# adthoms/dcora

Hardware: AMD Instinct MI355X
Metric: RBCD iterations/sec, sphere2500 5-agent split (higher is better)
Workload: dtype f64

## Files before the change

### dcora_amd/capi.py

```python
import ctypes as C
import os
import subprocess

import numpy as np

_HERE = os.path.dirname(os.path.abspath(__file__))
LIB_PATH = os.path.join(_HERE, "lib", "libdcora_hip.so")
HEADER_PATH = os.path.join(os.path.dirname(_HERE), "include", "dcora_hip.h")


class DcoraError(RuntimeError):
    def __init__(self, status, msg):
        super().__init__("dcora status %d: %s" % (status, msg))
        self.status = status


class Dims(C.Structure):
    _fields_ = [("r", C.c_int), ("d", C.c_int), ("n", C.c_int), ("l", C.c_int), ("b", C.c_int), ("layout", C.c_int)]


LAYOUT_AUTO, LAYOUT_SE, LAYOUT_RA = 0, 1, 2


class ROptParams(C.Structure):
# ... 167 lines not shown
    "dcora_exchange_info": (C.c_int, [_vp, _dp]),
    "dcora_exchange_link_report": (C.c_int, [_vp, _dp]),
    "dcora_exchange_post": (C.c_int, [_vp, _ip, C.c_int]),
    "dcora_exchange_wait": (C.c_int, [_vp, _ip, C.c_int]),
    "dcora_exchange_evaluate": (C.c_int, [_vp, _PD, _PD, _vp, _PI]),
    "dcora_exchange_rbcd_iterate": (C.c_int, [_vp, C.c_int, _PD, _PD, _vp, _PI]),
    "dcora_exchange_rbcd_tick": (C.c_int, [_vp, _ip, C.c_int, C.c_int]),
    "dcora_exchange_run_coloured": (C.c_int, [_vp, C.c_int, C.c_double, _PI, _vp, _vp]),
    "dcora_exchange_set_X": (C.c_int, [_vp, _dp]),
    "dcora_exchange_gather_X": (C.c_int, [_vp, _dp]),
    "dcora_exchange_barrier": (C.c_int, [_vp]),
    "dcora_exchange_all_ready": (C.c_int, [_vp, C.c_int, _PI]),
    "dcora_exchange_update_weights": (C.c_int, [_vp, C.c_int, _vp]),
    "dcora_exchange_set_weights": (C.c_int, [_vp, _dp]),
    "dcora_exchange_get_weights": (C.c_int, [_vp, _dp]),
    "dcora_exchange_certify": (C.c_int, [_vp, C.c_int, _vp, _vp, _vp, C.c_double, _PI, _PD, _PD, _dp,
                                         C.POINTER(C.c_longlong), _PI]),
    "dcora_exchange_host_selftest": (C.c_int, [C.c_char_p, C.c_int, C.c_int, C.c_int, C.c_int, _PD]),
    "dcora_debug_exchange_leave_stale": (C.c_int, [C.c_char_p, C.c_int, C.c_int]),
    "dcora_debug_exchange_probe_fault": (C.c_int, [C.c_int]),
    "dcora_cert_prepare": (C.c_int, [C.POINTER(Dims), _ip, _ip, C.c_int, C.c_int]),
    "dcora_debug_tcg_run_fault": (C.c_int, [C.c_int]),
    "dcora_debug_tcg_run_fault_at": (C.c_int, [C.c_int, C.c_int]),
    "dcora_problem_solver_info": (C.c_int, [_vp, _dp]),
    "dcora_ra_rbcd_create": (C.c_int, [_vp, C.POINTER(RbcdOptions), C.POINTER(_vp)]),
    "dcora_ra_rbcd_destroy": (C.c_int, [_vp]),
    "dcora_ra_rbcd_info": (C.c_int, [_vp, _PI, _vp]),
    "dcora_ra_rbcd_set_X": (C.c_int, [_vp, _dp]),
    "dcora_ra_rbcd_get_X": (C.c_int, [_vp, _dp]),
    "dcora_ra_rbcd_iterate": (C.c_int, [_vp, C.c_int, _PD, _PD, _vp, _PI]),
    "dcora_ra_rbcd_evaluate": (C.c_int, [_vp, _PD, _PD, _vp, _PI]),
    "dcora_ra_rbcd_run": (C.c_int, [_vp, C.c_int, C.c_double, _PI, _vp, _vp, _vp]),
    "dcora_ra_rbcd_iterate_set": (C.c_int, [_vp, _ip, C.c_int, C.c_int]),
    "dcora_ra_rbcd_set_acceleration": (C.c_int, [_vp, C.c_int]),
    "dcora_ra_rbcd_agent_colours": (C.c_int, [_vp, _ip, _PI]),
    "dcora_ra_rbcd_run_coloured": (C.c_int, [_vp, C.c_int, C.c_double, _PI, _vp, _vp]),
    "dcora_ra_rbcd_last_result": (C.c_int, [_vp, C.POINTER(ROptResult)]),
    "dcora_problem_time_qapply": (C.c_int, [_vp, C.c_int, _PD, _PD]),
    "dcora_problem_time_qapply_rotating": (C.c_int, [C.POINTER(_vp), C.c_int, C.c_int, _PD]),
    "dcora_problem_qapply_info": (C.c_int, [_vp, _dp]),
    "dcora_problem_time_precond": (C.c_int, [_vp, C.c_int, _PD, _PD]),
    "dcora_problem_precond_info": (C.c_int, [_vp, _dp]),
    "dcora_precond_cache_info": (C.c_int, [_dp]),
    "dcora_precond_cache_clear": (C.c_int, []),
    "dcora_robust_params_default": (None, [C.POINTER(RobustParams)]),
    "dcora_robust_weights": (C.c_int, [C.POINTER(RobustParams), C.c_int, C.c_int, _dp, _dp]),
# ... 58 lines not shown
```

### dcora_amd/csrc/capi.hip

```cpp
#include <cstdio>
#include <cstring>
#include <new>

#include "../../include/dcora_hip.h"
#include "cert.h"
#include "device_chol.h"
#include "device_problem.h"
#include "host_graph.h"
#include "host_threads.h"
#include "ra_rbcd.h"
#include "rbcd.h"
#include "precond_cache.h"
#include "exchange.h"
#include "host_robust.h"
#include "robust.h"
#include "round.h"

namespace dcora {
const std::string &get_last_error();
}
using namespace dcora;

struct dcora_problem_s {
  DeviceProblem p;
// ... 245 lines not shown
    info[2] = P.has_bsr ? (double)P.Qb.nblocks : 0.0;
    info[3] = P.has_bsr ? P.Qb.nblocks * (8.0 * (P.m.d + 1) * (P.m.d + 1) + 4.0) + 4.0 * (P.m.n + 1)
                        : 12.0 * P.Q.nnz + 4.0 * (P.m.k + 1);
    return DCORA_OK;
  });
}

int dcora_problem_solver_info(dcora_problem_t p, double *info) {
  return abi_call({p, info}, [&]() -> int {
    const DeviceProblem &P = p->p;
    info[0] = !P.use_pc() ? 0 : (P.tcg_run_ok ? 2 : 1);
    return DCORA_OK;
  });
}
int dcora_debug_tcg_run_fault(int runs) {
  g_tcg_run_fault_skip.store(0);
  g_tcg_run_fault.store(runs < 0 ? 0 : runs);
  return DCORA_OK;
}
int dcora_debug_tcg_run_fault_at(int skip, int runs) {
  g_tcg_run_fault_skip.store(skip < 0 ? 0 : skip);
  g_tcg_run_fault.store(runs < 0 ? 0 : runs);
  return DCORA_OK;
}
int dcora_problem_time_precond(dcora_problem_t p, int reps, double *avg_ms, double *bytes) {
  return abi_call({p, avg_ms, bytes}, [&] { return p->p.time_precond(reps, avg_ms, bytes); });
}
int dcora_problem_precond_info(dcora_problem_t p, double *info) {
  return abi_call({p, info}, [&]() -> int {
    const DeviceProblem &P = p->p;
    info[0] = !P.has_precond ? 0 : (P.sparse_precond ? 2 : 1);
    info[1] = !P.has_precond ? 0 : (P.sparse_precond ? P.sp.launches() : 1);
    info[2] = (double)P.precond_nnzL;
    info[3] = P.precond_setup_ms;
    info[4] = !P.has_precond ? 0 : (P.sparse_precond ? P.sp.weights_per_apply : (double)P.m.k * P.m.k);
    return DCORA_OK;
  });
}

int dcora_debug_sparse_weights_digest(dcora_problem_t p, double *out4) {
  return abi_call({p, out4}, [&]() -> int {
    const DeviceProblem &P = p->p;
    if (!P.sparse_precond || !P.sp.im) return bad("the problem has no sparse preconditioner");
    const DevBuf<double> &v = P.sp.im->vals;
    std::vector<double> h(v.n);
    DCORA_HIP(hipSetDevice(P.device));
// ... 1472 lines not shown
```

### dcora_amd/csrc/kernels.h

```cpp
#pragma once
#include <hip/hip_runtime.h>

#include <atomic>
#include <climits>
#include <vector>

namespace dcora {

constexpr int kMaxPartials = 1024;
constexpr int kBsrMaxGrid = 4096;
constexpr int kBlock = 256;
constexpr int kSpmmTile = 1536;

struct ManiDesc {
  int r, d, n, l, b, k, se;
  __host__ __device__ int rot_col(int i) const { return se ? i * (d + 1) : i * d; }
  __host__ __device__ int sphere_col(int i) const { return d * n + i; }
  __host__ __device__ int num_euc() const { return se ? n : n + b; }
  __host__ __device__ int euc_col(int e) const { return se ? e * (d + 1) + d : d * n + l + e; }
};
inline ManiDesc make_mani(int r, int d, int n, int l, int b, int layout = 0) {
  ManiDesc m;
  m.r = r; m.d = d; m.n = n; m.l = l; m.b = b;
  m.se = (layout == 2) ? 0 : ((l == 0 && b == 0) ? 1 : 0);
// ... 159 lines not shown
bool fused_supported(const ManiDesc &m);
bool group_supported(const ManiDesc &m);
int fused_pose_blocks(const ManiDesc &m);
int fused_nsplit(const ManiDesc &m);
int fused_precond_grid(const ManiDesc &m);
int fused_update_grid(const ManiDesc &m);
int launch_fused_hess(hipStream_t st, const ManiDesc &m, const CsrDev &Q, const double *z, const double *d_old,
                       double *d_new, Buf2 X, Buf2 S, double *Hd, const double *p3, int np3, double *p1,
                       SolverCtl *ctl, int seq, int iter,
                      const BsrDev *Ab = nullptr );
void launch_fused_precond(hipStream_t st, const ManiDesc &m, int ldm, const double *Minv, Buf2 grad,
                          const double *delta, const double *Hd, double *eta, double *Heta, const double *res_old,
                          double *res_new, double *Zpart, const double *p1, int np1, double *p2, SolverCtl *ctl,
                          HostFlags *hf, int seq, int iter, int first, SpFold sf = SpFold());
int fused_pc_blocks(const ManiDesc &m);
bool tcg_run_supported(const ManiDesc &m, int ldm, int cus, int max_rows_nnz);
int tcg_run_sync_words();
extern std::atomic<int> g_tcg_run_fault;
extern std::atomic<int> g_tcg_run_fault_skip;
int tcg_run_max_rows_nnz(const ManiDesc &m, const int *rowptr);
int launch_tcg_run(hipStream_t st, const ManiDesc &m, int ldm, const double *Minv, const CsrDev &Q, Buf2 grad, Buf2 X,
                   Buf2 S, double *d0, double *d1, double *Hd, double *eta, double *Heta, double *z, double *p1r,
                   double *p3, double *pC, unsigned *sync, SolverCtl *ctl, HostFlags *hf, int seq);
bool fused_pc_preferred(const ManiDesc &m, int ldm);
bool fused_pc_ready(const ManiDesc &m, int ldm);
int launch_fused_pc(hipStream_t st, const ManiDesc &m, int ldm, const double *Minv, Buf2 grad, Buf2 X,
                    const double *delta, const double *Hd, double *eta, double *Heta, const double *res_old,
                    double *res_new, double *z, const double *p1, int np1, double *p3, SolverCtl *ctl, HostFlags *hf,
                    int seq, int iter, int first, double *pC = nullptr );
void launch_fused_finish(hipStream_t st, const ManiDesc &m, Buf2 X, const double *Zpart, const double *res,
                         double *z, const double *p2, int np2, double *p3, SolverCtl *ctl, HostFlags *hf, int seq,
                         int iter, int first, int nsplit = -1 , SpFold sf = SpFold(),
                         double *zraw = nullptr );
int launch_fused_grad_bsr(hipStream_t st, int r, int d, const BsrDev &A, Buf2 X, const double *G, Buf2 EG, Buf2 RG, Buf2 S,
                          int sel, double *pA, double *pB, double *posenorm, Gate g,
                          const int *agent_start = nullptr, int agents = 0, int *wg_per_agent = nullptr);
int launch_fused_grad(hipStream_t st, const ManiDesc &m, const CsrDev &Q, Buf2 X, const double *G, Buf2 EG, Buf2 RG,
                      Buf2 Sblk, int sel, double *pA, double *pB, double *posenorm, Gate g,
                      const GradRide *ride = nullptr);
int launch_g_rgrad(hipStream_t st, const ManiDesc &m, Buf2 X, Buf2 EG, Buf2 RG, Buf2 Sblk, int sel, double *partials,
                   double *posenorm, Gate g);
void launch_ctl_init(hipStream_t st, SolverCtl *c, double tol, double Delta, double maxDelta, int max_outer,
                     int stop_on_accept, int max_inner);
void launch_eval_finish(hipStream_t st, int R, const int *pose_start, const double *posenorm, const double *pA,
                        int npA, EvalOut *out_dev, int seq, double *split_scratch = nullptr, int nposes = 0,
                        const double *agent_partials = nullptr, int wg_per_agent = 0);
// ... 84 lines not shown
```

### dcora_amd/csrc/solver_fused.hip

```cpp
#include <algorithm>
#include <stdexcept>
#include <atomic>
#include <type_traits>
#include <vector>
#include <cstdlib>
#include <cstring>

#include "kernels.h"
#include "tcg_rules.h"

namespace dcora {

namespace {

constexpr int GW = 8;

__device__ __forceinline__ double f_partial4_load(const double *__restrict__ p, int np) {
  const int l = (int)(threadIdx.x & 63u);
  const double a = (l < np) ? p[l] : 0.0, b = (l + 64 < np) ? p[l + 64] : 0.0;
  const double c = (l + 128 < np) ? p[l + 128] : 0.0, d = (l + 192 < np) ? p[l + 192] : 0.0;
  return (a + b) + (c + d);
}
__device__ __forceinline__ int f_partial_index(int np) { return np <= 64 ? (int)(threadIdx.x & 63u) : (int)threadIdx.x; }
__device__ __forceinline__ double f_partial_total(double v, int np, double *sm) {
// ... 904 lines not shown
  for (int a = 0; a < DH; ++a) acc += Zr.e[a] * Rr.e[a];
  const double tot = block_sum(acc, s_red);
  if (threadIdx.x == 0) p3[blockIdx.x] = tot;
  if (blockIdx.x == 0 && threadIdx.x == 0) {
    if (!first && iter + 1 >= c_max_inner) tcg_end_run_at_cap(ctl, hf, seq, iter + 1);
    host_store(&hf->last_seq_done, seq);
  }
}

typedef unsigned pc_v4u __attribute__((ext_vector_type(4)));
__device__ __forceinline__ double2 pc_ld16(__amdgpu_buffer_rsrc_t rs, unsigned voff, unsigned soff) {
  const pc_v4u v = __builtin_amdgcn_raw_buffer_load_b128(rs, voff, soff, 0);
  return __builtin_bit_cast(double2, v);
}
__device__ __forceinline__ double row16_sum_dpp(double v) {
  v += dpp_move<0xB1>(v);
  v += dpp_move<0x4E>(v);
  v += dpp_move<0x141>(v);
  v += dpp_move<0x140>(v);
  return v;
}
constexpr int kPcBlock = 256;
constexpr int kPcNW = kPcBlock / 64;
constexpr int kPcSB = 25;
constexpr int kPcLoads = 32;

template <int D, int PB, int R, bool MULTI>
__global__ __launch_bounds__(kPcBlock) void k_fused_pc(ManiDesc m, int ldm, int chk, const double *__restrict__ Minv,
                                                       Buf2 gradb, Buf2 Xb, const double *__restrict__ delta,
                                                       const double *__restrict__ Hd, double *__restrict__ eta,
                                                       double *__restrict__ Heta, const double *__restrict__ res_old,
                                                       double *__restrict__ res_new, double *__restrict__ z,
                                                       const double *__restrict__ p1, int np1,
                                                       double *__restrict__ p3, SolverCtl *ctl, HostFlags *hf, int seq,
                                                       int iter, int first, double *__restrict__ pC) {
  constexpr int DH = D + 1, NR = PB * DH, RM = R ? R : 8;
  constexpr int MB = kPcLoads / NR;
  extern __shared__ double s_res[];
  __shared__ double s_P[NR * RM + 1][4 * kPcNW];
  __shared__ double s_Z[NR * RM + 1], s_R[NR * RM];
  __shared__ double s_red[16];
  const int par = iter & 1;
  const int st_o = ctl->outer_done_stamp, st_t = ctl->tcg_done_stamp, cur = ctl->cur & 1;
  const double c_zr = ctl->z_r[par], c_dPd = ctl->d_Pd[par], c_ePe = ctl->e_Pe[par], c_ePd = ctl->e_Pd[par],
               c_Delta = ctl->Delta, c_ngf = ctl->ngf, c_n0 = ctl->norm_r0;
  const int c_max_inner = ctl->max_inner;
// ... 257 lines not shown

constexpr int kRunShards = 32, kRunCopies = 64, kRunStride = 32;
constexpr int kRunSyncWords = (kRunShards + 1 + kRunCopies + 1) * kRunStride;
constexpr int kRunQCap = 1024;
struct TcgRunArgs {
  ManiDesc m;
  int ldm;
  const double *Minv;
  CsrDev Q;
  Buf2 grad, X, S;
  double *d0, *d1, *Hd, *eta, *Heta, *z, *p1r, *p3, *pC;
  unsigned *sync;
  SolverCtl *ctl;
  HostFlags *hf;
  int seq, pbA;
  int fault;
#ifdef DCORA_RUN_STAMPS
  long long *stamps;
#endif
};
#ifdef DCORA_RUN_STAMPS
#define RUN_STAMP(i)                                                            \
  do {                                                                          \
    if (a.stamps && blockIdx.x == 0 && threadIdx.x == 0 && (i) < 64) a.stamps[(i)] = wall_clock64(); \
  } while (0)
#else
#define RUN_STAMP(i) \
  do {                \
  } while (0)
#endif
__device__ __forceinline__ double ld_coh(const double *p) {
  return __hip_atomic_load(p, __ATOMIC_RELAXED, __HIP_MEMORY_SCOPE_AGENT);
}
__device__ __forceinline__ void st_coh(double *p, double v) {
  __hip_atomic_store(p, v, __ATOMIC_RELAXED, __HIP_MEMORY_SCOPE_AGENT);
}
__device__ __forceinline__ double2 pc_ld16_coh(__amdgpu_buffer_rsrc_t rs, unsigned voff, unsigned soff) {
  const pc_v4u v = __builtin_amdgcn_raw_buffer_load_b128(rs, voff, soff, 16);
  return __builtin_bit_cast(double2, v);
}
constexpr unsigned kRunAbortBit = 0x80000000u;
__device__ __forceinline__ bool run_grid_step(unsigned *sync, unsigned step, int *s_ok) {
  __builtin_amdgcn_s_waitcnt(0);
  __syncthreads();
  if (threadIdx.x == 0) {
    unsigned *shard = sync, *top = sync + kRunShards * kRunStride, *done = top + kRunStride,
             *abort_w = done + kRunCopies * kRunStride;
    const int i = blockIdx.x, G = gridDim.x, sh = i % kRunShards;
    const unsigned in_shard = (unsigned)((G - sh + kRunShards - 1) / kRunShards), want = step + 1;
    const unsigned shards_used = (unsigned)(G < kRunShards ? G : kRunShards);
    const unsigned a = __hip_atomic_fetch_add(shard + sh * kRunStride, 1u, __ATOMIC_RELAXED, __HIP_MEMORY_SCOPE_AGENT);
    if (a + 1 == want * in_shard) {
      const unsigned b = __hip_atomic_fetch_add(top, 1u, __ATOMIC_RELAXED, __HIP_MEMORY_SCOPE_AGENT);
// ... 25 lines not shown
                                                     __HIP_MEMORY_SCOPE_AGENT)) {
              gave_up = true;
              break;
            }
          }
          if (gave_up) {
            __hip_atomic_store(abort_w, 1u, __ATOMIC_RELAXED, __HIP_MEMORY_SCOPE_AGENT);
            ok = 0;
            break;
          }
          t0 = wall_clock64();
        }
      }
    }
    *s_ok = ok;
  }
  __syncthreads();
  return *s_ok != 0;
}

template <int D, int R, int NS>
__global__ __launch_bounds__(kPcBlock) void k_tcg_run(TcgRunArgs a) {
  constexpr int DH = D + 1, PB = 2, NR = PB * DH, RM = R;
  extern __shared__ double s_res[];
  __shared__ double s_P[NR * RM + 1][4 * kPcNW];
  __shared__ double s_Z[NR * RM + 1], s_R[NR * RM], s_W[NR * RM], s_D[NR * RM], s_H[NR * RM];
  __shared__ double s_red[16];
  __shared__ int s_ci[kRunQCap];
  __shared__ double s_v[kRunQCap];
  __shared__ int s_ok;
  SolverCtl *ctl = a.ctl;
  const int seq = a.seq;
  RUN_STAMP(0);
  const int st_o = ctl->outer_done_stamp, cur = ctl->cur & 1;
  if (seq > st_o) return;
  const double c_Delta = ctl->Delta, c_ngf = ctl->ngf;
  const int c_max_inner = ctl->max_inner;
  const ManiDesc m = a.m;
  constexpr int r = R;
  const int k = m.k, ldm = a.ldm;
  const int pose0 = blockIdx.x * PB;
  const int npose = min(PB, m.n - pose0);
  const int j0 = pose0 * DH, nrow = npose * DH;
  const int wave = threadIdx.x >> 6, lane = threadIdx.x & 63;
  const int wave_u = __builtin_amdgcn_readfirstlane(wave);
  const int e = threadIdx.x;
  const bool own = e < nrow * r;
  const size_t oown = (size_t)j0 * r + e;
  const int lc = e / r, t = e - lc * r;
  const int g = threadIdx.x >> 3, tt = threadIdx.x & (GW - 1);
  const bool pact = (g < npose) && (tt < r);
  const size_t o = (size_t)(pose0 + min(g, npose - 1)) * DH * r;
  const double *__restrict__ grad = a.grad.p[cur];
  const double *__restrict__ X = a.X.p[cur];
  const unsigned vec_bytes = (unsigned)((size_t)r * k * sizeof(double));
  const __amdgpu_buffer_rsrc_t rs_g = __builtin_amdgcn_make_buffer_rsrc(const_cast<double *>(grad), 0, vec_bytes, 0x00020000);
  const __amdgpu_buffer_rsrc_t rs_h = __builtin_amdgcn_make_buffer_rsrc(a.Hd, 0, vec_bytes, 0x00020000);
  const __amdgpu_buffer_rsrc_t rs_m = __builtin_amdgcn_make_buffer_rsrc(
      const_cast<double *>(a.Minv), 0, (unsigned)((size_t)k * ldm * sizeof(double)), 0x00020000);
  const unsigned voff_t = threadIdx.x * 16u, voff_l = (unsigned)lane * 16u;
  double2 mreg[NS][NR];
#pragma unroll
  for (int u = 0; u < NS; ++u)
#pragma unroll
    for (int q = 0; q < NR; ++q)
      mreg[u][q] = pc_ld16(rs_m, voff_l, (unsigned)(((size_t)(j0 + q) * ldm + (size_t)(wave_u + kPcNW * u) * 128) * 8));
  double2 xg[kPcSB];
#pragma unroll
  for (int u = 0; u < kPcSB; ++u) xg[u] = pc_ld16(rs_g, voff_t, (unsigned)u * kPcBlock * 16u);
  const int pbeg = a.Q.rp[j0], pend = a.Q.rp[j0 + nrow];
  for (int i = threadIdx.x; i < pend - pbeg; i += kPcBlock) {
    s_ci[i] = a.Q.ci[pbeg + i];
    s_v[i] = a.Q.v[pbeg + i];
  }
  const int myb = own ? a.Q.rp[j0 + lc] - pbeg : 0, mye = own ? a.Q.rp[j0 + lc + 1] - pbeg : 0;
  Row<D> Y;
  ld_row<D>(X + o, r, tt, pact, Y);
  double S[D][D];
  {
    const double *__restrict__ Sblk = a.S.p[cur];
#pragma unroll
    for (int aa = 0; aa < D; ++aa)
#pragma unroll
      for (int b = 0; b < D; ++b) S[aa][b] = (g < npose) ? Sblk[(size_t)(pose0 + g) * D * D + aa + b * D] : 0.0;
  }
  double o_r = own ? grad[oown] : 0.0, o_eta = 0, o_Heta = 0, o_d = 0, o_h = 0;
  const int cpad = ((k + 127) / 128) * 128;
  const long Nc = (long)k * r;
  const int npair = (int)((Nc + 1) >> 1);
  const int nstep = cpad / 128;
  double zr = 0, dPd = 0, ePe = 0, ePd = 0, alpha = 0, ePen = 0;
  const double n0 = c_ngf;
  int status = TR_MAXITER, iters_done = 0;
  unsigned gstep = 0;
  double acc[NR][RM];
  double nrm2 = 0;
  auto product = [&]() {
#pragma unroll
    for (int q = 0; q < NR; ++q)
#pragma unroll
      for (int tq = 0; tq < RM; ++tq) acc[q][tq] = 0;
#pragma unroll
    for (int u = 0; u < NS; ++u) {
      const int sidx = wave_u + kPcNW * u;
      if (sidx < nstep) {
        const double *__restrict__ xs = s_res + (size_t)(sidx * 128 + 2 * lane) * r;
        double x0[RM], x1[RM];
#pragma unroll
        for (int tq = 0; tq < RM; ++tq) {
          x0[tq] = xs[tq];
          x1[tq] = xs[r + tq];
        }
#pragma unroll
        for (int tq = 0; tq < RM; ++tq)
#pragma unroll
          for (int q = 0; q < NR; ++q) acc[q][tq] = fma(x0[tq], mreg[u][q].x, fma(x1[tq], mreg[u][q].y, acc[q][tq]));
      }
    }
#pragma unroll
    for (int q = 0; q < NR; ++q)
#pragma unroll
      for (int tq = 0; tq < RM; ++tq) {
        const double v = row16_sum_dpp(acc[q][tq]);
        if ((lane & 15) == 0) s_P[q * RM + tq][wave * 4 + (lane >> 4)] = v;
      }
    {
      const double v = row16_sum_dpp(nrm2);
      if ((lane & 15) == 0) s_P[NR * RM][wave * 4 + (lane >> 4)] = v;
    }
    __syncthreads();
    if ((int)threadIdx.x <= NR * RM) {
      double v = 0;
#pragma unroll
      for (int w = 0; w < 4 * kPcNW; ++w) v += s_P[threadIdx.x][w];
      s_Z[threadIdx.x] = v;
    }
    __syncthreads();
  };
  auto project_z = [&]() {
    if (wave == 0) {
      Row<D> Zr, Rr;
#pragma unroll
      for (int aa = 0; aa < DH; ++aa) {
        Zr.e[aa] = pact ? s_Z[(g * DH + aa) * RM + tt] : 0.0;
        Rr.e[aa] = pact ? s_R[(g * DH + aa) * RM + tt] : 0.0;
      }
      row_tangent<D>(Y, Zr);
      if (pact)
#pragma unroll
        for (int aa = 0; aa < DH; ++aa) st_coh(a.z + o + aa * r + tt, Zr.e[aa]);
      double zacc = 0;
#pragma unroll
      for (int aa = 0; aa < DH; ++aa) zacc += Zr.e[aa] * Rr.e[aa];
      const double tot = wave_sum(zacc);
      if (lane == 0) st_coh(a.p3 + blockIdx.x, tot);
    }
  };
  auto finish = [&]() {
    if (blockIdx.x == 0 && threadIdx.x == 0) {
      ctl->alpha = alpha;
// ... 31 lines not shown
      a.pC[2 * blockIdx.x + 1] = t1;
    }
  };
  auto give_up = [&]() {
    if (threadIdx.x == 0) {
      ctl->outer_done_stamp = seq - 1;
      host_store(&a.hf->tcg_abort_seq, seq);
    }
  };
#pragma unroll
  for (int u = 0; u < kPcSB; ++u) {
    const int i = u * kPcBlock + (int)threadIdx.x;
    if (i < npair) {
      const double2 x = xg[u];
      nrm2 = fma(x.x, x.x, nrm2);
      nrm2 = fma(x.y, x.y, nrm2);
      reinterpret_cast<double2 *>(s_res)[i] = x;
    }
  }
  for (long i = 2L * npair + threadIdx.x; i < (long)cpad * r; i += kPcBlock) s_res[i] = 0.0;
  if (own) s_R[lc * RM + t] = o_r;
  __syncthreads();
  RUN_STAMP(1);
  product();
  project_z();
  RUN_STAMP(2);
  if (c_max_inner <= 0) {
    status = TR_MAXITER;
    finish();
    return;
  }
  if (a.fault && blockIdx.x == 0) return;
  if (!run_grid_step(a.sync, gstep++, &s_ok)) return give_up();
  RUN_STAMP(3);
  for (int iter = 0;; ++iter) {
    const int par = iter & 1;
    double *__restrict__ d_new = par ? a.d1 : a.d0;
    const double *__restrict__ d_old = par ? a.d0 : a.d1;
    {
      constexpr int kRunGB = 24;
      double ga[kRunGB], gz[kRunGB];
      double z_own = 0;
      if (own) {
        z_own = ld_coh(a.z + oown);
#pragma unroll
        for (int q = 0; q < kRunGB; ++q) {
          const bool ok = myb + q < mye;
          const size_t oo = ok ? (size_t)s_ci[myb + q] * r + t : 0;
          gz[q] = ld_coh(a.z + oo);
          ga[q] = (iter > 0) ? ld_coh(d_old + oo) : 0.0;
        }
      }
      const int np3 = gridDim.x;
      const int l = lane;
      const double pa = (l < np3) ? ld_coh(a.p3 + l) : 0.0, pb = (l + 64 < np3) ? ld_coh(a.p3 + l + 64) : 0.0;
      const double pcc = (l + 128 < np3) ? ld_coh(a.p3 + l + 128) : 0.0, pd = (l + 192 < np3) ? ld_coh(a.p3 + l + 192) : 0.0;
      const double z_r_new = wave_sum((pa + pb) + (pcc + pd));
      double beta = 0;
      if (iter > 0) beta = tcg_beta(z_r_new, zr);
      const TcgDir dir = iter == 0 ? tcg_dir_start(z_r_new) : tcg_dir_next(z_r_new, beta, alpha, dPd, ePd);
      zr = dir.z_r;
      ePd = dir.e_Pd;
      dPd = dir.d_Pd;
      ePe = iter == 0 ? 0.0 : ePen;
      double accw = 0, dn = 0;
      if (own) {
#pragma unroll
        for (int q = 0; q < kRunGB; ++q) {
          const double w = (myb + q < mye) ? s_v[myb + q] : 0.0;
          accw += w * (beta * ga[q] - gz[q]);
        }
        for (int p = myb + kRunGB; p < mye; p += 8) {
          double a8[8], b8[8], w8[8];
#pragma unroll
          for (int q = 0; q < 8; ++q) {
            const bool ok = p + q < mye;
            const size_t oo = ok ? (size_t)s_ci[p + q] * r + t : 0;
            w8[q] = ok ? s_v[p + q] : 0.0;
            b8[q] = ld_coh(a.z + oo);
            a8[q] = (iter > 0) ? ld_coh(d_old + oo) : 0.0;
// ... 13 lines not shown
#pragma unroll
        for (int aa = 0; aa < DH; ++aa) {
          W.e[aa] = pact ? s_W[(g * DH + aa) * r + tt] : 0.0;
          V.e[aa] = pact ? s_D[(g * DH + aa) * r + tt] : 0.0;
        }
        row_sub_AS<D>(W, V, S);
        row_tangent<D>(Y, W);
        if (pact)
#pragma unroll
          for (int aa = 0; aa < DH; ++aa) {
            st_coh(a.Hd + o + aa * r + tt, W.e[aa]);
            s_H[(g * DH + aa) * r + tt] = W.e[aa];
          }
        double dacc = 0;
#pragma unroll
        for (int aa = 0; aa < DH; ++aa) dacc += V.e[aa] * W.e[aa];
        if (!pact) dacc = 0;
        const double rs = row16_sum_dpp(dacc);
        if (lane == 0) st_coh(a.p1r + blockIdx.x, rs);
      }
      __syncthreads();
      if (own) o_h = s_H[e];
    }
    RUN_STAMP(4 + 7 * iter);
    if (!run_grid_step(a.sync, gstep++, &s_ok)) return give_up();
    RUN_STAMP(5 + 7 * iter);
    double2 xh[kPcSB];
#pragma unroll
    for (int u = 0; u < kPcSB; ++u) xh[u] = pc_ld16_coh(rs_h, voff_t, (unsigned)u * kPcBlock * 16u);
    double d_Hd;
    {
      const int rows_per = a.pbA / 2, nrows = gridDim.x, nblk = (nrows + rows_per - 1) / rows_per;
      double part = 0;
      if (lane < nblk) {
        const int b0 = lane * rows_per;
        double wsum[4] = {0, 0, 0, 0};
#pragma unroll
        for (int w = 0; w < 4; ++w) {
          double rs4[4];
#pragma unroll
          for (int q = 0; q < 4; ++q) {
            const int ri = w * 4 + q;
            rs4[q] = (ri < rows_per && b0 + ri < nrows) ? ld_coh(a.p1r + b0 + ri) : 0.0;
          }
          wsum[w] = (rs4[0] + rs4[1]) + (rs4[2] + rs4[3]);
        }
        double tsum = 0;
#pragma unroll
        for (int w = 0; w < 4; ++w) tsum += wsum[w];
// ... 2 lines not shown
      d_Hd = wave_sum(part);
    }
    const double c_zr = zr, c_dPd = dPd, c_ePe = ePe, c_ePd = ePd;
    alpha = tcg_alpha(c_zr, d_Hd);
    const double e_Pe_new = tcg_e_Pe_new(alpha, c_dPd, c_ePe, c_ePd);
    const bool boundary = tcg_boundary(d_Hd, e_Pe_new, c_Delta);
    const double step = boundary ? tcg_tau(c_dPd, c_ePe, c_ePd, c_Delta) : alpha;
    ePen = e_Pe_new;
    if (own) {
      o_eta = o_eta + step * o_d;
      o_Heta = o_Heta + step * o_h;
    }
    if (boundary) {
      status = tcg_boundary_status(d_Hd);
      iters_done = iter + 1;
      finish();
      return;
    }
    if (own) {
      const double rr = fma(alpha, o_h, o_r);
      o_r = rr;
      s_R[lc * RM + t] = rr;
    }
    RUN_STAMP(6 + 7 * iter);
    nrm2 = 0;
#pragma unroll
    for (int u = 0; u < kPcSB; ++u) {
      const int i = u * kPcBlock + (int)threadIdx.x;
      if (i < npair) {
        double2 x = reinterpret_cast<double2 *>(s_res)[i];
        x.x = fma(alpha, xh[u].x, x.x);
        x.y = fma(alpha, xh[u].y, x.y);
        nrm2 = fma(x.x, x.x, nrm2);
        nrm2 = fma(x.y, x.y, nrm2);
        reinterpret_cast<double2 *>(s_res)[i] = x;
      }
    }
    __syncthreads();
    RUN_STAMP(7 + 7 * iter);
    product();
    RUN_STAMP(8 + 7 * iter);
    {
      if (tcg_residual_done(sqrt(s_Z[NR * RM]), n0)) {
        status = tcg_residual_status(n0);
        iters_done = iter + 1;
        finish();
        return;
      }
    }
    project_z();
    if (iter + 1 >= c_max_inner) {
      iters_done = iter + 1;
      finish();
      return;
    }
    RUN_STAMP(9 + 7 * iter);
    if (!run_grid_step(a.sync, gstep++, &s_ok)) return give_up();
    RUN_STAMP(10 + 7 * iter);
  }
}


template <int D>
__global__ __launch_bounds__(kBlock) void k_g_rgrad(ManiDesc m, Buf2 Xb, Buf2 EGb, Buf2 RGb, Buf2 Sb, int sel,
                                                    double *__restrict__ partials, double *__restrict__ posenorm,
                                                    Gate g) {
  if (gated(g.ctl, g.seq, g.gate)) return;
  __shared__ double s_red[16];
  constexpr int DH = D + 1;
  const int idx = g.ctl ? ((g.ctl->cur ^ sel) & 1) : 0;
  const double *__restrict__ X = Xb.p[idx];
  const double *__restrict__ EG = EGb.p[idx];
  double *__restrict__ RG = RGb.p[idx];
  double *__restrict__ Sblk = Sb.p[idx];
  const int r = m.r;
  const int t = threadIdx.x & (GW - 1);
  double acc = 0;
  for (int pose0 = blockIdx.x * kPosesPerBlock; pose0 < m.n; pose0 += gridDim.x * kPosesPerBlock) {
    const int pose = pose0 + (threadIdx.x >> 3);
    const bool active = (pose < m.n) && (t < r);
    const size_t o = (size_t)pose * DH * r;
    Row<D> Y, E;
    ld_row<D>(X + o, r, t, active, Y);
    ld_row<D>(EG + o, r, t, active, E);
// ... 710 lines not shown
  int fault = 0;
  bool skipped = false;
  for (int sk = g_tcg_run_fault_skip.load(); sk > 0;)
    if (g_tcg_run_fault_skip.compare_exchange_weak(sk, sk - 1)) {
      skipped = true;
      break;
    }
  for (int left = skipped ? 0 : g_tcg_run_fault.load(); left > 0;)
    if (g_tcg_run_fault.compare_exchange_weak(left, left - 1)) {
      fault = 1;
      break;
    }
  TcgRunArgs a{m, ldm, Minv, Q, grad, X, S, d0, d1, Hd, eta, Heta, z, p1r, p3, pC, sync, ctl, hf, seq,
               fused_pb(m.r, m.d + 1), fault};
#ifdef DCORA_RUN_STAMPS
  {
    static long long *buf = nullptr;
    if (!buf) (void)hipHostMalloc((void **)&buf, 64 * sizeof(long long), hipHostMallocMapped);
    static int count = 0;
    if (buf && count > 0) {
      static double acc[64];
      static int n = 0;
      long long s0 = buf[0];
      if (buf[3] > s0 && buf[5 + 7 * 3] > 0) {
        for (int i = 0; i < 40; ++i) acc[i] += (double)(buf[i] - s0) * 0.01;
        ++n;
      }
      for (int i = 0; i < 64; ++i) buf[i] = 0;
      if (n == 500) {
        fprintf(stderr, "k_tcg_run stamps (us from start, workgroup 0, mean of %d runs with >= 4 iterations):", n);
        for (int i = 0; i < 34; ++i) fprintf(stderr, " %.2f", acc[i] / n);
        fprintf(stderr, "\n");
        n = -1000000;
      }
    }
    ++count;
    a.stamps = buf;
  }
#endif
  if (m.r == 4) return tcg_run_launch<4>(st, a);
  if (m.r == 5) return tcg_run_launch<5>(st, a);
  if (m.r == 6) return tcg_run_launch<6>(st, a);
  return -1;
}
int launch_fused_pc(hipStream_t st, const ManiDesc &m, int ldm, const double *Minv, Buf2 grad, Buf2 X,
                    const double *delta, const double *Hd, double *eta, double *Heta, const double *res_old,
                    double *res_new, double *z, const double *p1, int np1, double *p3, SolverCtl *ctl, HostFlags *hf,
                    int seq, int iter, int first, double *pC) {
  count_launch();
  return fused_pc_dispatch(st, m, ldm, Minv, grad, X, delta, Hd, eta, Heta, res_old, res_new, z, p1, np1, p3, ctl, hf,
                           seq, iter, first, pC, false);
}
bool fused_pc_ready(const ManiDesc &m, int ldm) {
  Buf2 none{};
  return fused_pc_dispatch(nullptr, m, ldm, nullptr, none, none, nullptr, nullptr, nullptr, nullptr, nullptr, nullptr,
                           nullptr, nullptr, 0, nullptr, nullptr, nullptr, 0, 0, 0, nullptr, true) >= 0;
}
void launch_fused_finish(hipStream_t st, const ManiDesc &m, Buf2 X, const double *Zpart, const double *res,
                         double *z, const double *p2, int np2, double *p3, SolverCtl *ctl, HostFlags *hf, int seq,
                         int iter, int first, int nsplit, SpFold sf, double *zraw) {
  const int grid = fused_pose_blocks(m);
  const int ns = nsplit > 0 ? nsplit : fused_nsplit(m);
  if (m.d == 3)
    hipLaunchKernelGGL(k_fused_finish<3>, dim3(grid), dim3(kBlock), 0, st, m, ns, X, Zpart, res, z, p2, np2, p3, ctl,
                       hf, seq, iter, first, sf, zraw);
  else
// ... 56 lines not shown
```

### include/dcora_hip.h

```cpp
#ifndef DCORA_HIP_H_
#define DCORA_HIP_H_

#ifdef __cplusplus
extern "C" {
#endif

typedef enum {
  DCORA_OK = 0,
  DCORA_ERR_BAD_ARG = 1,
  DCORA_ERR_NO_DEVICE = 2,
  DCORA_ERR_HIP = 3,
  DCORA_ERR_NOT_PD = 4,
  DCORA_ERR_NO_CONVERGENCE = 5,
  DCORA_ERR_NO_PRECONDITIONER = 6,
  DCORA_ERR_IO = 7,
  DCORA_ERR_UNSUPPORTED = 8,
  DCORA_ERR_EXCHANGE_LINK = 9
} dcora_status;

const char *dcora_status_string(int status);
const char *dcora_last_error(void);
int dcora_device_count(void);

enum {
// ... 23 lines not shown
void dcora_ropt_params_default(dcora_ropt_params *p);

typedef struct {
  int success;
  double fInit, gradNormInit, fOpt, gradNormOpt, elapsedMs;
  int tCGStatus;
  int outer_iterations, inner_iterations, accepted_steps;
} dcora_ropt_result;

typedef struct dcora_problem_s *dcora_problem_t;

int dcora_problem_create(const dcora_dims *dims, const int *rowptr, const int *colidx, const double *vals,
                         const double *G, double precond_reg, int device, dcora_problem_t *out);
int dcora_problem_destroy(dcora_problem_t p);
int dcora_problem_set_linear_term(dcora_problem_t p, const double *G);
int dcora_problem_cost(dcora_problem_t p, const double *X, double *f);
int dcora_problem_eucgrad(dcora_problem_t p, const double *X, double *out);
int dcora_problem_riegrad(dcora_problem_t p, const double *X, double *out, double *norm);
int dcora_problem_hessvec(dcora_problem_t p, const double *X, const double *V, double *out);
int dcora_debug_hessvec_solver_form(dcora_problem_t p, const double *X, const double *V, double *out, double *dots);
int dcora_problem_solver_info(dcora_problem_t p, double *info);
int dcora_debug_tcg_run_fault(int runs);
int dcora_debug_tcg_run_fault_at(int skip, int runs);
int dcora_problem_precondition(dcora_problem_t p, const double *X, const double *V, double *out);
int dcora_problem_retract(dcora_problem_t p, const double *X, const double *V, double *out);
int dcora_problem_tangent_project(dcora_problem_t p, const double *X, const double *V, double *out);
int dcora_problem_escape_saddle(dcora_problem_t p, const double *Xopt, double theta, const double *v,
                                double gradient_tolerance, double preconditioned_gradient_tolerance,
                                int is_second_order, double *Xout, int *success);
int dcora_manifold_project(const dcora_dims *dims, const double *M, double *out, int device);

int dcora_optimizer_optimize(dcora_problem_t p, const dcora_ropt_params *params, const double *X0, double *Xout,
                             dcora_ropt_result *result);

typedef struct dcora_csr_s *dcora_csr_t;
int dcora_csr_info(dcora_csr_t m, int *n, int *nnz);
int dcora_csr_copy(dcora_csr_t m, int *rowptr, int *colidx, double *vals);
int dcora_csr_destroy(dcora_csr_t m);

int dcora_cert_dual_matrix(const dcora_dims *dims, const double *X, const int *rowptr, const int *colidx,
                           const double *vals, int device, dcora_csr_t *S);
int dcora_cert_is_psd(int k, const int *rowptr, const int *colidx, const double *vals, int block, int *is_psd);
int dcora_cert_is_psd_device(int k, const int *rowptr, const int *colidx, const double *vals, int block, int device,
                             int *is_psd, double *info8);
int dcora_chol_host_selftest(int k, const int *rowptr, const int *colidx, const double *vals, int block, int *is_pd,
                             double *resid, double *info4);
// ... 237 lines not shown
```

Measured before the change: 4330.

## Replace per-value DPP row sums with permlane-swap transpose reduction in tCG run

The product step in the persistent tCG kernel used to reduce each of NR*RM+1 accumulators separately with a 16-lane DPP butterfly. It now uses a transpose-style reduction: permlane32/permlane16 swaps pair up values so each step halves the number of live values, then a short DPP finish. To make this work, shared-memory row reads use a permuted logical lane and double2 loads. The goal is fewer cross-lane ops and fewer shared-memory partial writes per product; the cost is a lane-permutation scheme that must stay consistent, which the added debug kernel and API are there to check. Timing stamps are also reorganised.

```diff
diff --git a/dcora_amd/capi.py b/dcora_amd/capi.py
--- a/dcora_amd/capi.py
+++ b/dcora_amd/capi.py
@@ -213,6 +213,7 @@
     "dcora_cert_prepare": (C.c_int, [C.POINTER(Dims), _ip, _ip, C.c_int, C.c_int]),
     "dcora_debug_tcg_run_fault": (C.c_int, [C.c_int]),
     "dcora_debug_tcg_run_fault_at": (C.c_int, [C.c_int, C.c_int]),
+    "dcora_debug_wg_sums": (C.c_int, [C.c_int, _dp, _dp]),
     "dcora_problem_solver_info": (C.c_int, [_vp, _dp]),
     "dcora_ra_rbcd_create": (C.c_int, [_vp, C.POINTER(RbcdOptions), C.POINTER(_vp)]),
     "dcora_ra_rbcd_destroy": (C.c_int, [_vp]),
diff --git a/dcora_amd/csrc/capi.hip b/dcora_amd/csrc/capi.hip
--- a/dcora_amd/csrc/capi.hip
+++ b/dcora_amd/csrc/capi.hip
@@ -291,6 +291,22 @@
   g_tcg_run_fault_skip.store(skip < 0 ? 0 : skip);
   g_tcg_run_fault.store(runs < 0 ? 0 : runs);
   return DCORA_OK;
+}
+int dcora_debug_wg_sums(int nv, const double *in, double *out) {
+  return abi_call({in, out}, [&]() -> int {
+    if (no_device()) return DCORA_ERR_NO_DEVICE;
+    if (nv != 33 && nv != 41 && nv != 49) return bad("dcora_debug_wg_sums: nv is 33, 41 or 49 (8 r + 1 at r = 4, 5, 6)");
+    const size_t nin = (size_t)nv * 256, nout = (size_t)2 * nv * 17;
+    DevBuf<double> I, O;
+    DCORA_HIP(I.alloc(nin));
+    DCORA_HIP(O.alloc(nout));
+    DCORA_HIP(hipMemcpy(I.p, in, nin * sizeof(double), hipMemcpyHostToDevice));
+    DCORA_HIP(hipMemset(O.p, 0, nout * sizeof(double)));
+    if (launch_debug_wg_sums(nullptr, nv, I.p, O.p) < 0) return bad("dcora_debug_wg_sums: the launch failed");
+    DCORA_HIP(hipDeviceSynchronize());
+    DCORA_HIP(hipMemcpy(out, O.p, nout * sizeof(double), hipMemcpyDeviceToHost));
+    return DCORA_OK;
+  });
 }
 int dcora_problem_time_precond(dcora_problem_t p, int reps, double *avg_ms, double *bytes) {
   return abi_call({p, avg_ms, bytes}, [&] { return p->p.time_precond(reps, avg_ms, bytes); });
diff --git a/dcora_amd/csrc/kernels.h b/dcora_amd/csrc/kernels.h
--- a/dcora_amd/csrc/kernels.h
+++ b/dcora_amd/csrc/kernels.h
@@ -205,6 +205,7 @@
 int launch_tcg_run(hipStream_t st, const ManiDesc &m, int ldm, const double *Minv, const CsrDev &Q, Buf2 grad, Buf2 X,
                    Buf2 S, double *d0, double *d1, double *Hd, double *eta, double *Heta, double *z, double *p1r,
                    double *p3, double *pC, unsigned *sync, SolverCtl *ctl, HostFlags *hf, int seq);
+int launch_debug_wg_sums(hipStream_t st, int nv, const double *in, double *out);
 bool fused_pc_preferred(const ManiDesc &m, int ldm);
 bool fused_pc_ready(const ManiDesc &m, int ldm);
 int launch_fused_pc(hipStream_t st, const ManiDesc &m, int ldm, const double *Minv, Buf2 grad, Buf2 X,
diff --git a/dcora_amd/csrc/solver_fused.hip b/dcora_amd/csrc/solver_fused.hip
--- a/dcora_amd/csrc/solver_fused.hip
+++ b/dcora_amd/csrc/solver_fused.hip
@@ -950,6 +950,40 @@
 }
 constexpr int kPcBlock = 256;
 constexpr int kPcNW = kPcBlock / 64;
+__device__ __forceinline__ int wg_sums_logical_lane(int p) { return ((p >> 5) & 1) | ((p >> 3) & 2) | ((p & 15) << 2); }
+template <bool HALF32>
+__device__ __forceinline__ double wg_sums_swap_add(double x, double y) {
+  typedef unsigned u2 __attribute__((ext_vector_type(2)));
+  u2 lo, hi;
+  if constexpr (HALF32) {
+    lo = __builtin_amdgcn_permlane32_swap((unsigned)__double2loint(x), (unsigned)__double2loint(y), false, false);
+    hi = __builtin_amdgcn_permlane32_swap((unsigned)__double2hiint(x), (unsigned)__double2hiint(y), false, false);
+  } else {
+    lo = __builtin_amdgcn_permlane16_swap((unsigned)__double2loint(x), (unsigned)__double2loint(y), false, false);
+    hi = __builtin_amdgcn_permlane16_swap((unsigned)__double2hiint(x), (unsigned)__double2hiint(y), false, false);
+  }
+  return __hiloint2double((int)hi[0], (int)lo[0]) + __hiloint2double((int)hi[1], (int)lo[1]);
+}
+template <int NV>
+__device__ __forceinline__ void wg_row_sums(const double (&v)[NV], double (*sP)[4 * kPcNW], int wave, int lane) {
+  constexpr int N1 = (NV + 1) / 2, N2 = (N1 + 1) / 2;
+  double a[N1], b[N2];
+#pragma unroll
+  for (int j = 0; j < N1; ++j) a[j] = wg_sums_swap_add<true>(v[2 * j], 2 * j + 1 < NV ? v[2 * j + 1] : 0.0);
+#pragma unroll
+  for (int j = 0; j < N2; ++j) {
+    double s = wg_sums_swap_add<false>(a[2 * j], 2 * j + 1 < N1 ? a[2 * j + 1] : 0.0);
+    s += dpp_move<0xB1>(s);
+    s += dpp_move<0x4E>(s);
+    b[j] = s;
+  }
+  if ((lane & 3) == 0) {
+    const int sub = ((lane >> 3) & 2) | (lane >> 5), slot = wave * 4 + ((lane >> 2) & 3);
+#pragma unroll
+    for (int j = 0; j < N2; ++j)
+      if (4 * j + sub < NV) sP[4 * j + sub][slot] = b[j];
+  }
+}
 constexpr int kPcSB = 25;
 constexpr int kPcLoads = 32;
 
@@ -1253,13 +1287,16 @@
 #ifdef DCORA_RUN_STAMPS
 #define RUN_STAMP(i)                                                            \
   do {                                                                          \
+    __builtin_amdgcn_sched_barrier(0);                                          \
     if (a.stamps && blockIdx.x == 0 && threadIdx.x == 0 && (i) < 64) a.stamps[(i)] = wall_clock64(); \
+    __builtin_amdgcn_sched_barrier(0);                                          \
   } while (0)
 #else
 #define RUN_STAMP(i) \
   do {                \
   } while (0)
 #endif
+constexpr int kRunStamp0 = 4, kRunStampsPerIter = 10;
 __device__ __forceinline__ double ld_coh(const double *p) {
   return __hip_atomic_load(p, __ATOMIC_RELAXED, __HIP_MEMORY_SCOPE_AGENT);
 }
@@ -1331,7 +1368,8 @@
 template <int D, int R, int NS>
 __global__ __launch_bounds__(kPcBlock) void k_tcg_run(TcgRunArgs a) {
   constexpr int DH = D + 1, PB = 2, NR = PB * DH, RM = R;
-  extern __shared__ double s_res[];
+  extern __shared__ __align__(16) double s_img[];
+  double *const s_res = s_img;
   __shared__ double s_P[NR * RM + 1][4 * kPcNW];
   __shared__ double s_Z[NR * RM + 1], s_R[NR * RM], s_W[NR * RM], s_D[NR * RM], s_H[NR * RM];
   __shared__ double s_red[16];
@@ -1367,7 +1405,12 @@
   const __amdgpu_buffer_rsrc_t rs_h = __builtin_amdgcn_make_buffer_rsrc(a.Hd, 0, vec_bytes, 0x00020000);
   const __amdgpu_buffer_rsrc_t rs_m = __builtin_amdgcn_make_buffer_rsrc(
       const_cast<double *>(a.Minv), 0, (unsigned)((size_t)k * ldm * sizeof(double)), 0x00020000);
-  const unsigned voff_t = threadIdx.x * 16u, voff_l = (unsigned)lane * 16u;
+#ifdef DCORA_RUN_BUTTERFLY_SUMS
+  const int llane = lane;
+#else
+  const int llane = wg_sums_logical_lane(lane);
+#endif
+  const unsigned voff_t = threadIdx.x * 16u, voff_l = (unsigned)llane * 16u;
   double2 mreg[NS][NR];
 #pragma unroll
   for (int u = 0; u < NS; ++u)
@@ -1402,41 +1445,43 @@
   const double n0 = c_ngf;
   int status = TR_MAXITER, iters_done = 0;
   unsigned gstep = 0;
-  double acc[NR][RM];
+  double acc[NR * RM + 1];
   double nrm2 = 0;
-  auto product = [&]() {
-#pragma unroll
-    for (int q = 0; q < NR; ++q)
-#pragma unroll
-      for (int tq = 0; tq < RM; ++tq) acc[q][tq] = 0;
+  auto product = [&](int sb) {
+#pragma unroll
+    for (int i = 0; i < NR * RM; ++i) acc[i] = 0;
 #pragma unroll
     for (int u = 0; u < NS; ++u) {
       const int sidx = wave_u + kPcNW * u;
       if (sidx < nstep) {
-        const double *__restrict__ xs = s_res + (size_t)(sidx * 128 + 2 * lane) * r;
-        double x0[RM], x1[RM];
+        const double2 *__restrict__ xs = reinterpret_cast<const double2 *>(s_img) + (size_t)(sidx * 64 + llane) * r;
+        double x[2 * RM];
 #pragma unroll
         for (int tq = 0; tq < RM; ++tq) {
-          x0[tq] = xs[tq];
-          x1[tq] = xs[r + tq];
+          const double2 xx = xs[tq];
+          x[2 * tq] = xx.x;
+          x[2 * tq + 1] = xx.y;
         }
 #pragma unroll
         for (int tq = 0; tq < RM; ++tq)
 #pragma unroll
-          for (int q = 0; q < NR; ++q) acc[q][tq] = fma(x0[tq], mreg[u][q].x, fma(x1[tq], mreg[u][q].y, acc[q][tq]));
-      }
-    }
-#pragma unroll
-    for (int q = 0; q < NR; ++q)
-#pragma unroll
-      for (int tq = 0; tq < RM; ++tq) {
-        const double v = row16_sum_dpp(acc[q][tq]);
-        if ((lane & 15) == 0) s_P[q * RM + tq][wave * 4 + (lane >> 4)] = v;
-      }
-    {
-      const double v = row16_sum_dpp(nrm2);
-      if ((lane & 15) == 0) s_P[NR * RM][wave * 4 + (lane >> 4)] = v;
-    }
+          for (int q = 0; q < NR; ++q)
+            acc[q * RM + tq] = fma(x[tq], mreg[u][q].x, fma(x[r + tq], mreg[u][q].y, acc[q * RM + tq]));
+      }
+    }
+    RUN_STAMP(sb);
+#ifdef DCORA_RUN_BUTTERFLY_SUMS
+    acc[NR * RM] = nrm2;
+#pragma unroll
+    for (int i = 0; i <= NR * RM; ++i) {
+      const double v = row16_sum_dpp(acc[i]);
+      if ((lane & 15) == 0) s_P[i][wave * 4 + (lane >> 4)] = v;
+    }
+#else
+    acc[NR * RM] = __shfl(nrm2, llane);
+    wg_row_sums<NR * RM + 1>(acc, s_P, wave, lane);
+#endif
+    RUN_STAMP(sb + 1);
     __syncthreads();
     if ((int)threadIdx.x <= NR * RM) {
       double v = 0;
@@ -1445,6 +1490,7 @@
       s_Z[threadIdx.x] = v;
     }
     __syncthreads();
+    RUN_STAMP(sb + 2);
   };
   auto project_z = [&]() {
     if (wave == 0) {
@@ -1522,7 +1568,7 @@
   if (own) s_R[lc * RM + t] = o_r;
   __syncthreads();
   RUN_STAMP(1);
-  product();
+  product(64);
   project_z();
   RUN_STAMP(2);
   if (c_max_inner <= 0) {
@@ -1535,6 +1581,7 @@
   RUN_STAMP(3);
   for (int iter = 0;; ++iter) {
     const int par = iter & 1;
+    [[maybe_unused]] const int sb0 = kRunStamp0 + kRunStampsPerIter * iter;
     double *__restrict__ d_new = par ? a.d1 : a.d0;
     const double *__restrict__ d_old = par ? a.d0 : a.d1;
     {
@@ -1556,6 +1603,10 @@
       const double pa = (l < np3) ? ld_coh(a.p3 + l) : 0.0, pb = (l + 64 < np3) ? ld_coh(a.p3 + l + 64) : 0.0;
       const double pcc = (l + 128 < np3) ? ld_coh(a.p3 + l + 128) : 0.0, pd = (l + 192 < np3) ? ld_coh(a.p3 + l + 192) : 0.0;
       const double z_r_new = wave_sum((pa + pb) + (pcc + pd));
+#ifdef DCORA_RUN_STAMPS
+      __builtin_amdgcn_s_waitcnt(0);
+      RUN_STAMP(sb0);
+#endif
       double beta = 0;
       if (iter > 0) beta = tcg_beta(z_r_new, zr);
       const TcgDir dir = iter == 0 ? tcg_dir_start(z_r_new) : tcg_dir_next(z_r_new, beta, alpha, dPd, ePd);
@@ -1615,9 +1666,9 @@
       __syncthreads();
       if (own) o_h = s_H[e];
     }
-    RUN_STAMP(4 + 7 * iter);
+    RUN_STAMP(sb0 + 1);
     if (!run_grid_step(a.sync, gstep++, &s_ok)) return give_up();
-    RUN_STAMP(5 + 7 * iter);
+    RUN_STAMP(sb0 + 2);
     double2 xh[kPcSB];
 #pragma unroll
     for (int u = 0; u < kPcSB; ++u) xh[u] = pc_ld16_coh(rs_h, voff_t, (unsigned)u * kPcBlock * 16u);
@@ -1666,7 +1717,7 @@
       o_r = rr;
       s_R[lc * RM + t] = rr;
     }
-    RUN_STAMP(6 + 7 * iter);
+    RUN_STAMP(sb0 + 3);
     nrm2 = 0;
 #pragma unroll
     for (int u = 0; u < kPcSB; ++u) {
@@ -1681,9 +1732,8 @@
       }
     }
     __syncthreads();
-    RUN_STAMP(7 + 7 * iter);
-    product();
-    RUN_STAMP(8 + 7 * iter);
+    RUN_STAMP(sb0 + 4);
+    product(sb0 + 5);
     {
       if (tcg_residual_done(sqrt(s_Z[NR * RM]), n0)) {
         status = tcg_residual_status(n0);
@@ -1698,12 +1748,45 @@
       finish();
       return;
     }
-    RUN_STAMP(9 + 7 * iter);
+    RUN_STAMP(sb0 + 8);
     if (!run_grid_step(a.sync, gstep++, &s_ok)) return give_up();
-    RUN_STAMP(10 + 7 * iter);
-  }
-}
-
+    RUN_STAMP(sb0 + 9);
+  }
+}
+
+template <int NV>
+__global__ __launch_bounds__(kPcBlock) void k_debug_wg_sums(const double *__restrict__ in, double *__restrict__ out) {
+  __shared__ double s_P[NV][4 * kPcNW];
+  const int wave = threadIdx.x >> 6, lane = threadIdx.x & 63;
+  double v[NV];
+#pragma unroll
+  for (int form = 0; form < 2; ++form) {
+    const int src = wave * 64 + (form == 0 ? wg_sums_logical_lane(lane) : lane);
+#pragma unroll
+    for (int i = 0; i < NV; ++i) v[i] = in[(size_t)i * kPcBlock + src];
+    if (form == 0) {
+      wg_row_sums<NV>(v, s_P, wave, lane);
+    } else {
+#pragma unroll
+      for (int i = 0; i < NV; ++i) {
+        const double s = row16_sum_dpp(v[i]);
+        if ((lane & 15) == 0) s_P[i][wave * 4 + (lane >> 4)] = s;
+      }
+    }
+    __syncthreads();
+    double *__restrict__ o = out + (size_t)form * NV * (4 * kPcNW + 1);
+    if ((int)threadIdx.x < NV) {
+      double t = 0;
+#pragma unroll
+      for (int w = 0; w < 4 * kPcNW; ++w) {
+        t += s_P[threadIdx.x][w];
+        o[threadIdx.x * 4 * kPcNW + w] = s_P[threadIdx.x][w];
+      }
+      o[NV * 4 * kPcNW + threadIdx.x] = t;
+    }
+    __syncthreads();
+  }
+}
 
 template <int D>
 __global__ __launch_bounds__(kBlock) void k_g_rgrad(ManiDesc m, Buf2 Xb, Buf2 EGb, Buf2 RGb, Buf2 Sb, int sel,
@@ -2460,14 +2543,15 @@
       static double acc[64];
       static int n = 0;
       long long s0 = buf[0];
-      if (buf[3] > s0 && buf[5 + 7 * 3] > 0) {
-        for (int i = 0; i < 40; ++i) acc[i] += (double)(buf[i] - s0) * 0.01;
+      constexpr int kShown = kRunStamp0 + 4 * kRunStampsPerIter;
+      if (buf[3] > s0 && buf[kShown - 1] > 0) {
+        for (int i = 0; i < kShown; ++i) acc[i] += (double)(buf[i] - s0) * 0.01;
         ++n;
       }
       for (int i = 0; i < 64; ++i) buf[i] = 0;
       if (n == 500) {
-        fprintf(stderr, "k_tcg_run stamps (us from start, workgroup 0, mean of %d runs with >= 4 iterations):", n);
-        for (int i = 0; i < 34; ++i) fprintf(stderr, " %.2f", acc[i] / n);
+        fprintf(stderr, "k_tcg_run stamps (us from start, workgroup 0, mean of %d runs that went past their fourth iteration):", n);
+        for (int i = 0; i < kShown; ++i) fprintf(stderr, " %.2f", acc[i] / n);
         fprintf(stderr, "\n");
         n = -1000000;
       }
@@ -2480,6 +2564,13 @@
   if (m.r == 5) return tcg_run_launch<5>(st, a);
   if (m.r == 6) return tcg_run_launch<6>(st, a);
   return -1;
+}
+int launch_debug_wg_sums(hipStream_t st, int nv, const double *in, double *out) {
+  if (nv == 33) hipLaunchKernelGGL((k_debug_wg_sums<33>), dim3(1), dim3(kPcBlock), 0, st, in, out);
+  else if (nv == 41) hipLaunchKernelGGL((k_debug_wg_sums<41>), dim3(1), dim3(kPcBlock), 0, st, in, out);
+  else if (nv == 49) hipLaunchKernelGGL((k_debug_wg_sums<49>), dim3(1), dim3(kPcBlock), 0, st, in, out);
+  else return -1;
+  return hipGetLastError() == hipSuccess ? 0 : -1;
 }
 int launch_fused_pc(hipStream_t st, const ManiDesc &m, int ldm, const double *Minv, Buf2 grad, Buf2 X,
                     const double *delta, const double *Hd, double *eta, double *Heta, const double *res_old,
diff --git a/include/dcora_hip.h b/include/dcora_hip.h
--- a/include/dcora_hip.h
+++ b/include/dcora_hip.h
@@ -69,6 +69,7 @@
 int dcora_problem_solver_info(dcora_problem_t p, double *info);
 int dcora_debug_tcg_run_fault(int runs);
 int dcora_debug_tcg_run_fault_at(int skip, int runs);
+int dcora_debug_wg_sums(int nv, const double *in, double *out);
 int dcora_problem_precondition(dcora_problem_t p, const double *X, const double *V, double *out);
 int dcora_problem_retract(dcora_problem_t p, const double *X, const double *V, double *out);
 int dcora_problem_tangent_project(dcora_problem_t p, const double *X, const double *V, double *out);
```

Result: faster. 4552 (median of 6 runs) (+5.1%).
